# UCSB-NLP-Chang/Diffusion-SpaceTime-Attn

Hardware: AMD Instinct MI355X
Metric: images/sec at 512x512, 50 PLMS steps, 2 objects (higher is better)
Workload: dtype fp16; 1 GPU; SD-v1-4 UNet+VAE (synthetic weights), 512x512, 50 PLMS steps (51 CFG UNet calls), 2 objects, fixed blend weights (BASELINE configs[1]); global_batch=64, parallelism=prompt-parallel dp1, hipgraph=True, linear_weights=fp16, trunk_layout=NHWC, weight_broadcast_bytes=0

## Files before the change

diffusion-spacetime-attn_amd/csrc/sta_rowgemm.hip:

```cpp

#include <hip/hip_runtime.h>
#include <stdint.h>
#include "sta_xattn.h"
#include "sta_internal.h"
#include "sta_xattn_dev.h"
#include "sta_wring_dev.h"
#include "sta_xattn_proj3.h"

namespace {

constexpr int RG_C = 320;
constexpr int RG_NKS = RG_C / 32;
constexpr int RG_NRT = RG_C / 16;
constexpr int RG_NCH = RG_NRT / 2;
constexpr int RG_NW = 8;
constexpr int RG_CHUNK_FR = 2 * RG_NKS;
using RgRing = WRing<RG_NW, RG_CHUNK_FR>;
constexpr int RG_SLOT = RgRing::SLOT;
constexpr int RG_TAB = 3 * RG_C * 2;
constexpr int RG_LDS = 2 * RG_SLOT + RG_TAB;

__host__ __device__ constexpr int sfrag_channel(int f, int g, int j) {
  return f < 8 ? f * 40 + (j < 4 ? 4 * g + j : 16 + 4 * g + (j - 4)) : (4 * (f - 8) + g) * 40 + 32 + j;
}
// ... 98 lines not shown
    const T* xr = (const T*)p.x + row * RG_C + 8 * g;
    V8 xv[RG_NCH];
#pragma unroll
    for (int v = 0; v < RG_NCH; ++v) xv[v] = *(const V8*)(xr + 32 * v);
    float sum = 0.f;
#pragma unroll
    for (int v = 0; v < RG_NCH; ++v) {
      const V8 bs = *(const V8*)(tab + 32 * v + 8 * g);
      V8 o;
#pragma unroll
      for (int e = 0; e < 8; ++e) {
        const float t = acc[2 * v + (e >> 2)][e & 3] + (float)bs[e] + (float)xv[v][e];
        o[e] = (T)t;
        const float r = (float)o[e];
        acc[2 * v + (e >> 2)][e & 3] = r;
        sum += r;
      }
      *(V8*)((T*)p.s + row * RG_C + 32 * v + 8 * g) = o;
      __builtin_amdgcn_sched_barrier(0);
    }
    const float mean = bfly_sum(sum) * (1.0f / RG_C);
    float q = 0.f;
#pragma unroll
    for (int u = 0; u < RG_NRT; ++u)
#pragma unroll
      for (int r = 0; r < 4; ++r) {
        const float d = acc[u][r] - mean;
        q += d * d;
      }
    const float rstd = rsqrtf(bfly_sum(q) * (1.0f / RG_C) + p.eps);
#pragma unroll
    for (int v = 0; v < RG_NCH; ++v) {
      const V8 gm = *(const V8*)(tab + RG_C + 32 * v + 8 * g), bt = *(const V8*)(tab + 2 * RG_C + 32 * v + 8 * g);
      V8 o;
#pragma unroll
      for (int e = 0; e < 8; ++e) o[e] = (T)((acc[2 * v + (e >> 2)][e & 3] - mean) * rstd * (float)gm[e] + (float)bt[e]);
      if (p.y_qfrag) *(V8*)((char*)p.y + (size_t)row0 * RG_C * sizeof(T) + v * FRAG + lane * 16) = o;
      else *(V8*)((T*)p.y + row * RG_C + 32 * v + 8 * g) = o;
      __builtin_amdgcn_sched_barrier(0);
    }
    }
  }
  asm volatile("s_waitcnt vmcnt(0)" ::: "memory");
}

}

extern "C" {

size_t sta_to_out_ln_packed_wo_bytes(int C, int heads) {
  return (C == RG_C && heads == 8) ? (size_t)RG_NRT * RG_NKS * FRAG : 0;
}

int sta_to_out_ln_pack_wo(const void* wo, void* packed, int C, int heads, int kind, int dtype, void* stream) {
  g_sta_err[0] = 0;
  if (!wo || !packed) return sta_fail(STA_E_ARG, "null pointer");
  if (sta_to_out_ln_packed_wo_bytes(C, heads) == 0) return sta_fail(STA_E_UNSUP, "to_out + LayerNorm in out-fragment order: C = 320 with 8 heads only (C=%d heads=%d)", C, heads);
  if (dtype != STA_BF16 && dtype != STA_F16) return sta_fail(STA_E_UNSUP, "dtype %d", dtype);
  if (kind != 0 && kind != 1) return sta_fail(STA_E_ARG, "fragment kind %d (0: cross-attention out fragments, 1: self-attention out fragments)", kind);
  hipStream_t st = (hipStream_t)stream;
  return sta_by_dtype(dtype, [&](auto tag) {
    using T = decltype(tag);
    return sta_launch<pack_wo_ofrag_kernel<T>>("pack_wo_ofrag launch", dim3(RG_NRT * RG_NKS), dim3(64), 0, st, (const T*)wo, (T*)packed, kind);
  });
}

int sta_to_out_ln_ofrag(const void* blended_ofrag, const void* packed_wo, const void* bias, const void* x, const void* gamma,
                        const void* beta, void* s, void* y, long R, int C, int heads, float eps, int y_qfrag, int dtype, void* stream) {
  g_sta_err[0] = 0;
  if (!blended_ofrag || !packed_wo || !x || !gamma || !beta || !s || !y) return sta_fail(STA_E_ARG, "null pointer");
  if (sta_to_out_ln_packed_wo_bytes(C, heads) == 0) return sta_fail(STA_E_UNSUP, "to_out + LayerNorm in out-fragment order: C = 320 with 8 heads only (C=%d heads=%d)", C, heads);
  if (R <= 0 || R % 16) return sta_fail(STA_E_ARG, "to_out_ln_ofrag: R=%ld (need a positive multiple of 16 rows)", R);
  if ((size_t)R * C * 2 >= 0xfffffff0ull) return sta_fail(STA_E_UNSUP, "activations must stay below 4 GiB (R=%ld)", R);
  RG p{(const char*)blended_ofrag, (const char*)packed_wo, bias, gamma, beta, x, s, y, R, eps, y_qfrag ? 1 : 0};
  const long nblk = (R + 16 * RG_NW - 1) / (16 * RG_NW);
  const unsigned grid = (unsigned)(nblk < 256 ? nblk : 256);
  hipStream_t st = (hipStream_t)stream;
  return sta_by_dtype(dtype, [&](auto tag) {
    return sta_launch_lds<to_out_ln_ofrag_kernel<decltype(tag)>>("to_out_ln_ofrag launch", RG_LDS, dim3(grid), dim3(64 * RG_NW), RG_LDS, st, p);
  });
}

}
```

diffusion-spacetime-attn_amd/sta/fused.py:

```python

import torch

from . import lib

_DT = {torch.bfloat16: lib.STA_BF16, torch.float16: lib.STA_F16}
ENABLED = True
_hold = 0
TRACKED = False


class held:

    def __enter__(self):
        global _hold
        _hold += 1

    def __exit__(self, *exc):
        global _hold
        _hold -= 1


class tracked:

    def __init__(self, on=True):
# ... 427 lines not shown
    nb = max(1, min(B, CONV_MAX_BYTES // per_in))
    L = lib.load()
    slots = L.sta_conv3x3_s2_stats_slots(H, W) if stats else 0
    part = torch.empty((B + 1, slots, Cout, 2), dtype=torch.float32, device=x.device) if slots else None
    for b0 in range(0, B, nb):
        n = min(nb, B - b0)
        lib.check(L.sta_conv3x3_s2_nhwc(x.data_ptr() + b0 * per_in, w_packed.data_ptr(), z.data_ptr(), _ptr(bias), out.data_ptr() + b0 * per_out,
                                        0 if part is None else part.data_ptr() + b0 * slots * Cout * 8, n, H, W, Cin, Cout, _DT[x.dtype],
                                        _stream()), "sta_conv3x3_s2_nhwc")
    if part is not None and _version(out) is not None:
        out._sta_stats = (out._version, _finalize_stats(part, B, slots, Cout))
    return out


def vae_encode_step(h, quant_weight, quant_bias, n_post, n_enc, scale_factor, sqrt_a, sqrt_1ma, want_z0=False, want_xin=True):
    B, C, Hh, Ww = h.shape
    if C != 8 or not h.is_cuda or h.dtype not in _DT:
        raise ValueError("vae_encode_step: 16-bit CUDA h [B, 8, h, w], got %s %s" % (tuple(h.shape), h.dtype))
    h = h.contiguous(memory_format=torch.channels_last)
    qw = quant_weight.detach().reshape(8, 8).float().contiguous()
    qb = quant_bias.detach().float().contiguous()
    f = lambda t: t.detach().to(device=h.device, dtype=torch.float32).contiguous()
    n_post, n_enc = f(n_post), f(n_enc)
    if n_post.shape != (B, 4, Hh, Ww) or n_enc.shape != (B, 4, Hh, Ww):
        raise ValueError("vae_encode_step: noises must be [B, 4, h, w] = %s" % ((B, 4, Hh, Ww),))
    x = torch.empty((B, 4, Hh, Ww), dtype=torch.float32, device=h.device)
    z0 = torch.empty_like(x) if want_z0 else None
    xin = torch.empty((2 * B, 4, Hh, Ww), dtype=h.dtype, device=h.device) if want_xin else None
    lib.check(lib.load().sta_vae_encode_step(h.data_ptr(), qw.data_ptr(), qb.data_ptr(), n_post.data_ptr(), n_enc.data_ptr(), x.data_ptr(),
                                             _ptr(z0), _ptr(xin), B, Hh * Ww, float(scale_factor), float(sqrt_a), float(sqrt_1ma), _DT[h.dtype],
                                             _stream()), "sta_vae_encode_step")
    return x, z0, xin


CAT_IN_PLACE = True


def groupnorm_silu_cat(xa, xb, weight, bias, groups, eps, silu=True):
    B, Ca = xa.shape[0], xa.shape[1]
    C = Ca + xb.shape[1]
    HW = xa.numel() // (B * Ca)
    L = lib.load()
    y = torch.empty((B, C) + tuple(xa.shape[2:]), dtype=xa.dtype, device=xa.device, memory_format=torch.channels_last)
    sa, sb = (_producer_stats(xa), _producer_stats(xb)) if GN_STATS_FROM_PRODUCER else (None, None)
    if sa is not None and sb is not None:
        lib.check(L.sta_groupnorm_silu_nhwc_cstats(xa.data_ptr(), xb.data_ptr(), Ca, sa.data_ptr(), sb.data_ptr(), None, weight.data_ptr(),
                                                   bias.data_ptr(), y.data_ptr(), B, C, HW, groups, float(eps), int(bool(silu)), _DT[xa.dtype],
                                                   _stream()), "sta_groupnorm_silu_nhwc_cstats")
        return y
    ws = torch.empty(L.sta_groupnorm_nhwc_workspace_bytes(B, HW, groups) // 4, dtype=torch.float32, device=xa.device)
    lib.check(L.sta_groupnorm_silu_nhwc_cat(xa.data_ptr(), xb.data_ptr(), Ca, None, weight.data_ptr(), bias.data_ptr(), y.data_ptr(),
                                            ws.data_ptr(), B, C, HW, groups, float(eps), int(bool(silu)), _DT[xa.dtype], _stream()),
              "sta_groupnorm_silu_nhwc_cat")
    return y


def cat_supported(xa, xb, groups, skip_weight):
    if not (CAT_IN_PLACE and usable(xa) and is_nhwc(xa) and is_nhwc(xb) and xa.dtype == xb.dtype and xa.shape[0] == xb.shape[0]
            and xa.shape[2:] == xb.shape[2:]):
        return False
    Ca, C = xa.shape[1], xa.shape[1] + xb.shape[1]
    if Ca % 64 or C % 8 or C % groups or (C // groups < 8 and C // groups != 4) or C > 4096 or groups > 64:
        return False
    rows = xa.numel() // Ca
    return (LINEAR_ROWS and rows >= LINEAR_MIN_ROWS and skip_weight.dtype == xa.dtype
            and bool(lib.load().sta_linear_rows_supported(rows, C, skip_weight.shape[0])))


def linear_rows_cat(xa, xb, w_packed, N, bias=None, res=None):
    Ka, Kb = xa.shape[-1], xb.shape[-1]
    R = xa.numel() // Ka
    assert xa.is_contiguous() and xb.is_contiguous() and xb.numel() // Kb == R and Ka % 64 == 0
    out = torch.empty(xa.shape[:-1] + (N,), dtype=xa.dtype, device=xa.device)
    if bias is not None:
        bias = bias.to(xa.dtype).contiguous()
    z = _zeros_page(xa.device, 2 * (Ka + Kb))
    lib.check(lib.load().sta_linear_rows_cat(xa.data_ptr(), xb.data_ptr(), Ka, w_packed.data_ptr(), z.data_ptr(), _ptr(bias), _ptr(res),
                                             out.data_ptr(), R, Ka + Kb, N, _DT[xa.dtype], _stream()), "sta_linear_rows_cat")
    return out


LINEAR_ROWS = True
LINEAR_MIN_ROWS = 4096


_retired_pages = []


def _zeros_page(device, nbytes):
    z = _conv_zeros.get(device)
    if z is None or z.numel() < nbytes:
        if z is not None:
            _retired_pages.append(z)
        z = _conv_zeros[device] = torch.zeros(max(nbytes, 16384), dtype=torch.uint8, device=device)
    return z


def linear_rows_supported(x, weight):
    if not (LINEAR_ROWS and x.is_cuda and x.dtype in _DT and not torch.is_grad_enabled() and ENABLED and not _hold and weight.dtype == x.dtype):
        return False
    K = x.shape[-1]
    R = x.numel() // K
    return R >= LINEAR_MIN_ROWS and x.is_contiguous() and bool(lib.load().sta_linear_rows_supported(R, K, weight.shape[0]))


def pack_linear_weight(weight):
    N, K = weight.shape[0], weight.shape[1]
    L = lib.load()
    n = L.sta_linear_rows_packed_w_bytes(K, N)
    if n == 0 or not weight.is_cuda:
        raise ValueError("linear_rows: a CUDA weight [N %% 160 == 0 or N %% 128 == 0, K %% 64 == 0]; got %s" % (tuple(weight.shape),))
    w = weight.detach()
    buf = torch.empty(n, dtype=torch.uint8, device=w.device)
    lib.check(L.sta_linear_rows_pack_w(w.data_ptr(), w.stride(0), w.stride(1), buf.data_ptr(), K, N, _DT[w.dtype], _stream()), "sta_linear_rows_pack_w")
    return buf


def linear_rows(x, w_packed, N, bias=None, res=None, stats_rows=None):
    K = x.shape[-1]
    R = x.numel() // K
    out = torch.empty(x.shape[:-1] + (N,), dtype=x.dtype, device=x.device)
    if res is not None:
        assert res.numel() == out.numel() and res.dtype == x.dtype and res.is_contiguous()
    if bias is not None:
        bias = bias.to(x.dtype).contiguous()
    z = _zeros_page(x.device, 2 * K)
    if stats_rows and stats_rows % 256 == 0 and R % stats_rows == 0:
        n_img, slots = R // stats_rows, stats_rows // 64
        part = torch.empty((n_img + 1, slots, N, 2), dtype=torch.float32, device=x.device)
        lib.check(lib.load().sta_linear_rows_stats(x.data_ptr(), w_packed.data_ptr(), z.data_ptr(), _ptr(bias), _ptr(res), out.data_ptr(),
                                                   part.data_ptr(), stats_rows, R, K, N, _DT[x.dtype], _stream()), "sta_linear_rows_stats")
        if _version(out) is not None:
            out._sta_stats = (out._version, _finalize_stats(part, n_img, slots, N))
        return out
    lib.check(lib.load().sta_linear_rows(x.data_ptr(), w_packed.data_ptr(), z.data_ptr(), _ptr(bias), _ptr(res), out.data_ptr(), R, K, N,
                                         _DT[x.dtype], _stream()), "sta_linear_rows")
    return out


def packed_linear_weight(owner, key_obj, weight):
    return cached_image(owner, ("linear", id(key_obj)), (weight,), lambda: pack_linear_weight(weight))


def linear_module(lin, x, res=None):
    if linear_rows_supported(x, lin.weight) and (res is None or res.is_contiguous()):
        return linear_rows(x, packed_linear_weight(lin, lin, lin.weight), lin.weight.shape[0], bias=lin.bias, res=res)
    y = torch.nn.functional.linear(x, lin.weight, lin.bias)
    return y if res is None else y + res


def add_bias_nchw(a, b=None, bias=None):
    B, C = a.shape[0], a.shape[1]
    HW = a.numel() // (B * C)
    if (C % 8 if is_nhwc(a) else HW % 8):
        t = a if b is None else a + b
        return t if bias is None else t + bias[None, :, None, None]
    y = torch.empty_like(a)
    if is_nhwc(a):
        if b is not None and not is_nhwc(b):
            b = b.contiguous(memory_format=torch.channels_last)
        lib.check(lib.load().sta_add_bias_rows(a.data_ptr(), _ptr(b), _ptr(bias), y.data_ptr(), B * HW, C, _DT[a.dtype], _stream()),
                  "sta_add_bias_rows")
        return y
    if b is not None and not b.is_contiguous():
        b = b.contiguous()
    lib.check(lib.load().sta_add_bias_nchw(a.data_ptr(), _ptr(b), _ptr(bias), y.data_ptr(), B, C, HW, _DT[a.dtype], _stream()),
              "sta_add_bias_nchw")
    return y


def tracked_usable(x):
    return (TRACKED and ENABLED and x.is_cuda and x.dtype in _DT and torch.is_grad_enabled()
            and (is_nhwc(x) if x.dim() == 4 else x.is_contiguous()))


class GroupNormSiLUFn(torch.autograd.Function):

    @staticmethod
    def forward(ctx, x, add, weight, bias, groups, eps, silu):
        B, C = x.shape[0], x.shape[1]
        HW = x.numel() // (B * C)
        L = lib.load()
        add = None if add is None else add.float().contiguous()
        y = torch.empty_like(x)
        ws = torch.empty(L.sta_groupnorm_nhwc_workspace_bytes(B, HW, groups) // 4, dtype=torch.float32, device=x.device)
        lib.check(L.sta_groupnorm_silu_nhwc(x.data_ptr(), _ptr(add), weight.data_ptr(), bias.data_ptr(), y.data_ptr(), ws.data_ptr(),
                                            B, C, HW, groups, float(eps), int(bool(silu)), _DT[x.dtype], _stream()), "sta_groupnorm_silu_nhwc")
        ctx.save_for_backward(x, add, weight, bias, ws)
        ctx.cfg = (B, C, HW, groups, float(eps), int(bool(silu)))
        return y

    @staticmethod
    def backward(ctx, dy):
        x, add, weight, bias, ws = ctx.saved_tensors
        B, C, HW, groups, eps, silu = ctx.cfg
        if not is_nhwc(dy):
            dy = dy.contiguous(memory_format=torch.channels_last)
        dx = torch.empty_like(x)
        wsb = torch.empty_like(ws)
        lib.check(lib.load().sta_groupnorm_silu_nhwc_bwd(x.data_ptr(), _ptr(add), weight.data_ptr(), bias.data_ptr(), dy.data_ptr(),
                                                         dx.data_ptr(), ws.data_ptr(), wsb.data_ptr(), B, C, HW, groups, eps, silu,
                                                         _DT[x.dtype], _stream()), "sta_groupnorm_silu_nhwc_bwd")
        return dx, None, None, None, None, None, None


def groupnorm_silu_tracked(x, weight, bias, groups, eps, add=None, silu=True):
    C = x.shape[1]
    if add is not None and add.requires_grad:
        raise RuntimeError("the pre-add of the fused GroupNorm carries no gradient (timestep embedding)")
    if not is_nhwc(x) or C % 8 or (C // groups < 8 and C // groups != 4) or C > 4096 or groups > 64:
        h = x if add is None else x + add.to(x.dtype)[:, :, None, None]
        h = torch.nn.functional.group_norm(h, groups, weight, bias, eps)
        return torch.nn.functional.silu(h) if silu else h
    return GroupNormSiLUFn.apply(x, add, weight, bias, groups, eps, silu)


class GegluFn(torch.autograd.Function):
    @staticmethod
    def forward(ctx, h):
        ctx.save_for_backward(h)
        return geglu(h)

    @staticmethod
    def backward(ctx, dy):
# ... 98 lines not shown
```

diffusion-spacetime-attn_amd/sta/lib.py:

```python
import ctypes
import glob
import os
import shutil
import subprocess

_HERE = os.path.dirname(os.path.abspath(__file__))
PKG_ROOT = os.path.dirname(_HERE)
REPO_ROOT = os.path.dirname(PKG_ROOT)
CSRC = os.path.join(PKG_ROOT, "csrc")
INCLUDE = os.path.join(REPO_ROOT, "include")
LIB_PATH = os.path.join(CSRC, "libsta_xattn.so")
SOURCES = [os.path.join(CSRC, n) for n in ("sta_xattn.hip", "sta_xattn_bwd.hip", "sta_xattn_proj.hip", "sta_xattn_proj3.hip", "sta_rowgemm.hip", "sta_ffgemm.hip", "sta_lnqkv.hip", "sta_conv.hip", "sta_gemm.hip", "sta_selfattn.hip", "sta_selfattn_bwd.hip", "sta_unet.hip", "sta_unet_bwd.hip", "sta_fp8.hip", "sta_mxfp8.hip", "sta_sampler.hip", "sta_encode.hip", "sta_clip.hip", "sta_inpaint.hip")]
INCLUDED_SOURCES = {"sta_xattn_maps_bwd.hip": "sta_xattn_bwd.hip", "sta_guide.hip": "sta_sampler.hip", "sta_window.hip": "sta_sampler.hip"}

PER_SOURCE_FLAGS = {"sta_selfattn.hip": ["-mllvm", "-amdgpu-mfma-vgpr-form", "-ffinite-math-only"],
                    "sta_selfattn_bwd.hip": ["-mllvm", "-amdgpu-mfma-vgpr-form", "-ffinite-math-only"],
                    "sta_xattn.hip": ["-ffinite-math-only"], "sta_xattn_bwd.hip": ["-ffinite-math-only"], "sta_xattn_proj.hip": ["-ffinite-math-only"],
                    "sta_xattn_proj3.hip": ["-ffinite-math-only"], "sta_rowgemm.hip": ["-ffinite-math-only"], "sta_ffgemm.hip": ["-ffinite-math-only"], "sta_conv.hip": ["-ffinite-math-only"], "sta_gemm.hip": ["-ffinite-math-only"]}

NO_SPILL_KERNELS = {"sta_ffgemm.hip": ("ff_geglu_qfrag_kernel",), "sta_conv.hip": ("ELb1EEEvNS_2CVE",),
                    "sta_sampler.hip": ("window_split_kernel", "window_fuse_kernel", "sampler_step_windows_kernel",
                                        "sampler_step_windows_masked_kernel", "window_blend_kernel")}

STA_BF16, STA_F16 = 0, 1
STA_MX8_GEGLU, STA_MX8_MX_OUT = 1, 2
OPT_FWD_KERNEL, OPT_STAGED_TILES, OPT_STAGED_WAVES, OPT_STAGED_QT, OPT_HEAD_MAJOR, OPT_SPLIT_QT, OPT_SELFATTN_32, OPT_PROJ_PAIR, OPT_SELFATTN_WAVES, OPT_SELFATTN_PIPE, OPT_PROJ_LL2, OPT_BWD_KERNEL, OPT_BWD_SLOTS, OPT_BWD_WAVES = range(14)
FWD_STAGED, FWD_SPLIT = 1, 2
MAX_KEYS, MAX_HEAD_DIM, MAX_OBJECTS = 80, 160, 8
P3_STATS_WORDS = 8
MAX_READOUTS = 16
MAX_WINDOW_OFFSETS, STA_SRC_F32 = 16, 2

_vp, _i, _f, _sz, _l = ctypes.c_void_p, ctypes.c_int, ctypes.c_float, ctypes.c_size_t, ctypes.c_long
SYMBOLS = {
    "sta_version": (_i, []),
    "sta_last_error": (ctypes.c_char_p, []),
    "sta_built_with": (ctypes.c_char_p, []),
    "sta_set_option": (_i, [_i, _i]),
    "sta_xattn_packed_kv_bytes": (_sz, [_i, _i, _i]),
    "sta_xattn_pack_kv": (_i, [_vp, _vp, _vp, _i, _i, _i, _i, _i, _vp]),
    "sta_xattn_fwd": (_i, [_vp, _vp, _vp, _vp, _vp, _vp, _i, _i, _i, _i, _i, _i, _f, _i, _vp]),
    "sta_xattn_token_maps": (_i, [_vp, _vp, _vp, _vp, _vp, _i, _i, _i, _i, _i, _i, _i, _f, _i, _i, _vp]),
    "sta_xattn_token_maps_bwd": (_i, [_vp, _vp, _vp, _vp, _vp, _vp, _i, _i, _i, _i, _i, _i, _i, _f, _i, _vp]),
    "sta_xattn_fwd_proj_supported": (_i, [_i, _i, _i, _i]),
    "sta_xattn_fwd_proj_locals_from_l2": (_i, [_i, _i, _i, _i]),
    "sta_xattn_packed_wq_bytes": (_sz, [_i, _i]),
    "sta_xattn_pack_wq": (_i, [_vp, _vp, _i, _i, _i, _vp]),
    "sta_xattn_packed_kv_proj_bytes": (_sz, [_i, _i, _i]),
    "sta_xattn_pack_kv_proj": (_i, [_vp, _vp, _vp, _i, _i, _i, _i, _i, _vp]),
    "sta_xattn_fwd_proj": (_i, [_vp, _vp, _vp, _vp, _vp, _vp, _i, _i, _i, _i, _i, _i, _f, _i, _vp]),
    "sta_xattn_fwd_proj_qfrag_supported": (_i, [_i, _i, _i, _i, _i, _i]),
    "sta_xattn_fwd_proj_ex": (_i, [_vp, _vp, _vp, _vp, _vp, _vp, _i, _i, _i, _i, _i, _i, _f, _i, _i, _vp, _vp]),
    "sta_xattn_fwd_proj_qfrag": (_i, [_vp, _vp, _vp, _vp, _vp, _vp, _i, _i, _i, _i, _i, _i, _f, _i, _vp]),
    "sta_xattn_fwd_proj_qfrag_ofrag": (_i, [_vp, _vp, _vp, _vp, _vp, _vp, _i, _i, _i, _i, _i, _i, _f, _i, _vp]),
    "sta_to_out_ln_packed_wo_bytes": (_sz, [_i, _i]),
    "sta_to_out_ln_pack_wo": (_i, [_vp, _vp, _i, _i, _i, _i, _vp]),
    "sta_to_out_ln_ofrag": (_i, [_vp, _vp, _vp, _vp, _vp, _vp, _vp, _vp, _l, _i, _i, _f, _i, _i, _vp]),
    "sta_selfattn_fwd_sfrag": (_i, [_vp, _vp, _vp, _vp, _i, _i, _i, _i, _i, _i, _l, _l, _f, _i, _vp]),
    "sta_xattn_bwd_workspace_bytes": (_sz, [_i, _i, _i, _i]),
    "sta_xattn_bwd": (_i, [_vp, _vp, _vp, _vp, _vp, _vp, _vp, _vp, _i, _i, _i, _i, _i, _i, _f, _i, _vp]),
    "sta_selfattn_fwd": (_i, [_vp, _vp, _vp, _vp, _i, _i, _i, _i, _i, _i, _l, _l, _f, _i, _vp]),
    "sta_selfattn_fwd_optimistic": (_i, [_vp, _vp, _vp, _vp, _vp, _i, _i, _i, _i, _i, _i, _l, _l, _f, _i, _i, _vp]),
    "sta_selfattn_optimistic_supported": (_i, [_i, _i, _i, _f, _i]),
    "sta_selfattn_optimistic_flags_bytes": (ctypes.c_size_t, [_i, _i, _i]),
    "sta_selfattn_fwd_lse": (_i, [_vp, _vp, _vp, _vp, _vp, _i, _i, _i, _i, _i, _i, _l, _l, _f, _i, _vp]),
    "sta_selfattn_bwd": (_i, [_vp] * 13 + [_i, _i, _i, _i, _i, _i, _f, _i, _vp]),
    "sta_groupnorm_silu": (_i, [_vp, _vp, _vp, _vp, _vp, _i, _i, _i, _i, _f, _i, _i, _vp]),
    "sta_geglu": (_i, [_vp, _vp, _l, _i, _i, _vp]),
    "sta_add_layernorm": (_i, [_vp, _vp, _vp, _vp, _vp, _vp, _vp, _l, _i, _f, _i, _vp]),
    "sta_add_layernorm_qfrag": (_i, [_vp, _vp, _vp, _vp, _vp, _vp, _vp, _l, _i, _f, _i, _vp]),
    "sta_ff_geglu_packed_w_bytes": (_sz, [_i, _i]),
    "sta_ff_geglu_pack_w": (_i, [_vp, _vp, _i, _i, _i, _vp]),
    "sta_ff_geglu_qfrag": (_i, [_vp, _vp, _vp, _vp, _l, _i, _i, _i, _i, _vp]),
    "sta_ff_geglu_c640_packed_w_bytes": (_sz, [_i, _i]),
    "sta_ff_geglu_c640_pack_w": (_i, [_vp, _vp, _i, _i, _i, _vp]),
    "sta_ff_geglu_c640_qfrag": (_i, [_vp, _vp, _vp, _vp, _l, _i, _i, _i, _i, _vp]),
    "sta_ff_out_packed_w_bytes": (_sz, [_i, _i]),
    "sta_ff_out_pack_w": (_i, [_vp, _vp, _i, _i, _i, _vp]),
    "sta_ff_out_res_hfrag": (_i, [_vp, _vp, _vp, _vp, _vp, _l, _i, _i, _i, _vp]),
    "sta_ln_qkv_packed_w_bytes": (_sz, [_i]),
    "sta_ln_qkv_pack_w": (_i, [_vp, _vp, _vp, _i, _i, _vp]),
    "sta_ln_qkv": (_i, [_vp] * 9 + [_l, _i, _f, _i, _vp]),
    "sta_conv3x3_nhwc_supported": (_i, [_i, _i, _i, _i, _i]),
    "sta_conv3x3_packed_w_bytes": (_sz, [_i, _i]),
    "sta_conv3x3_pack_w": (_i, [_vp, _l, _l, _l, _l, _vp, _i, _i, _i, _vp]),
    "sta_conv3x3_nhwc": (_i, [_vp, _vp, _vp, _vp, _vp, _vp, _vp, _i, _i, _i, _i, _i, _i, _i, _vp]),
    "sta_conv3x3_up2_nhwc_supported": (_i, [_i, _i, _i, _i, _i]),
    "sta_conv3x3_up2_stats_slots": (_i, [_i, _i]),
    "sta_conv3x3_up2_packed_w_bytes": (_sz, [_i, _i]),
    "sta_conv3x3_up2_pack_w": (_i, [_vp, _l, _l, _l, _l, _vp, _i, _i, _i, _vp]),
    "sta_conv3x3_up2_nhwc": (_i, [_vp, _vp, _vp, _vp, _vp, _vp, _vp, _i, _i, _i, _i, _i, _i, _vp]),
    "sta_linear_rows_supported": (_i, [_l, _i, _i]),
    "sta_linear_rows_packed_w_bytes": (_sz, [_i, _i]),
    "sta_linear_rows_pack_w": (_i, [_vp, _l, _l, _vp, _i, _i, _i, _vp]),
    "sta_linear_rows": (_i, [_vp, _vp, _vp, _vp, _vp, _vp, _l, _i, _i, _i, _vp]),
    "sta_conv3x3_stats_slots": (_i, [_i, _i]),
    "sta_stats_finalize": (_i, [_vp, _vp, _i, _i, _i, _vp]),
    "sta_linear_rows_stats": (_i, [_vp, _vp, _vp, _vp, _vp, _vp, _vp, _l, _l, _i, _i, _i, _vp]),
    "sta_groupnorm_silu_nhwc_cstats": (_i, [_vp, _vp, _i, _vp, _vp, _vp, _vp, _vp, _vp, _i, _i, _i, _i, _f, _i, _i, _vp]),
    "sta_linear_rows_cat": (_i, [_vp, _vp, _i, _vp, _vp, _vp, _vp, _vp, _l, _i, _i, _i, _vp]),
    "sta_groupnorm_silu_nhwc_cat": (_i, [_vp, _vp, _i, _vp, _vp, _vp, _vp, _vp, _i, _i, _i, _i, _f, _i, _i, _vp]),
    "sta_add_bias_nchw": (_i, [_vp, _vp, _vp, _vp, _i, _i, _i, _i, _vp]),
    "sta_groupnorm_nhwc_workspace_bytes": (_sz, [_i, _i, _i]),
    "sta_groupnorm_silu_nhwc": (_i, [_vp, _vp, _vp, _vp, _vp, _vp, _i, _i, _i, _i, _f, _i, _i, _vp]),
    "sta_add_bias_rows": (_i, [_vp, _vp, _vp, _vp, _l, _i, _i, _vp]),
    "sta_quant_rows_fp8": (_i, [_vp, _vp, _vp, _l, _i, _i, _vp]),
    "sta_mx8_quant_rows": (_i, [_vp, _vp, _vp, _l, _i, _i, _vp]),
    "sta_mx8_gemm": (_i, [_vp, _vp, _vp, _vp, _vp, _vp, _vp, _vp, _l, _i, _i, _l, _i, _i, _vp]),
    "sta_groupnorm_silu_nhwc_bwd": (_i, [_vp, _vp, _vp, _vp, _vp, _vp, _vp, _vp, _i, _i, _i, _i, _f, _i, _i, _vp]),
    "sta_geglu_bwd": (_i, [_vp, _vp, _vp, _l, _i, _i, _vp]),
    "sta_layernorm_bwd": (_i, [_vp, _vp, _vp, _vp, _vp, _l, _i, _f, _i, _vp]),
    "sta_sampler_step": (_i, [_vp] * 7 + [_l, _l] + [_f] * 8 + [_i, _vp]),
    "sta_sampler_step_bwd": (_i, [_vp] * 5 + [_l, _l] + [_f] * 7 + [_i, _vp]),
    "sta_conv3x3_s2_nhwc_supported": (_i, [_i, _i, _i, _i, _i]),
    "sta_conv3x3_s2_stats_slots": (_i, [_i, _i]),
    "sta_conv3x3_s2_nhwc": (_i, [_vp] * 6 + [_i] * 6 + [_vp]),
    "sta_vae_encode_step": (_i, [_vp] * 8 + [_l, _l, _f, _f, _f, _i, _vp]),
    "sta_clip_views": (_i, [_vp] * 4 + [_i] * 5 + [_vp]),
    "sta_clip_views_bwd": (_i, [_vp] * 4 + [_i] * 5 + [_vp]),
    "sta_sampler_step_masked": (_i, [_vp] * 10 + [_l, _l, _l] + [_f] * 10 + [_i, _vp]),
    "sta_sampler_step_masked_bwd": (_i, [_vp] * 6 + [_l, _l, _l] + [_f] * 7 + [_i, _vp]),
    "sta_latent_blend": (_i, [_vp] * 6 + [_l, _l, _l, _f, _f, _i, _vp]),
    "sta_image_composite": (_i, [_vp] * 4 + [_l, _l, _i, _vp]),
    "sta_image_composite_bwd": (_i, [_vp] * 4 + [_l, _l, _i, _vp]),
    "sta_latent_guide": (_i, [_vp] * 7 + [_l, _l, _l, _i, _f, _i, _vp]),
    "sta_window_split": (_i, [_vp, _vp, _l] + [_i] * 6 + [_vp, _vp] + [_i] * 3 + [_vp]),
    "sta_window_fuse": (_i, [_vp, _vp, _l] + [_i] * 5 + [_vp, _vp, _i, _i, _vp]),
    "sta_sampler_step_windows": (_i, [_vp] * 7 + [_l] + [_i] * 5 + [_vp, _vp, _i] + [_f] * 8 + [_i, _vp]),
    "sta_sampler_step_windows_masked": (_i, [_vp] * 10 + [_l] + [_i] * 5 + [_vp, _vp, _i] + [_f] * 10 + [_i, _vp]),
    "sta_window_blend": (_i, [_vp] * 6 + [_l] + [_i] * 5 + [_vp, _vp, _i, _f, _f, _i, _vp]),
}


class StaLibraryError(RuntimeError):
    pass


def _stale():
    if not os.path.exists(LIB_PATH):
        return True
    t = os.path.getmtime(LIB_PATH)
    deps = SOURCES + [os.path.join(CSRC, n) for n in INCLUDED_SOURCES] + [os.path.join(_HERE, "isa_lint.py")] + glob.glob(os.path.join(INCLUDE, "*.h")) + glob.glob(os.path.join(CSRC, "*.h"))
    return any(os.path.exists(d) and os.path.getmtime(d) > t for d in deps)


LINT_LOG = os.path.join(CSRC, ".isa_lint.log")


def _llvm_bin(hipcc):
    for root in (os.environ.get("ROCM_PATH"), os.path.dirname(os.path.dirname(os.path.realpath(hipcc))), "/opt/rocm"):
        if root and os.path.exists(os.path.join(root, "lib", "llvm", "bin", "clang")):
            return os.path.join(root, "lib", "llvm", "bin")
    raise StaLibraryError("no lib/llvm/bin/clang beside %s (set ROCM_PATH)" % hipcc)


def _hipcc_headline(hipcc):
    ver = subprocess.run([hipcc, "--version"], capture_output=True, text=True).stdout.strip().splitlines()
    return ver[0] if ver else "hipcc ?"


def _run(cmd):
    r = subprocess.run(cmd, capture_output=True, text=True)
    if r.returncode != 0:
        raise StaLibraryError("build step failed: %s\n%s" % (" ".join(cmd), r.stdout + r.stderr))


_META_KEYS = ("vgpr_count", "vgpr_spill_count", "sgpr_spill_count", "private_segment_fixed_size", "group_segment_fixed_size")


def kernel_metadata(text):
    out, cur, inside = {}, None, False
    for line in text.splitlines():
        if line.startswith("amdhsa.kernels:"):
            inside = True
        elif inside and line[:1] not in (" ", ""):
            inside = False
        if not inside:
            continue
# ... 148 lines not shown
```

include/sta_unet.h:

```cpp
#ifndef STA_UNET_H
#define STA_UNET_H

#include <stddef.h>
#include <stdint.h>

#ifdef __cplusplus
extern "C" {
#endif

int sta_groupnorm_silu(const void* x, const float* add, const void* gamma, const void* beta, void* y,
                       int B, int C, int HW, int G, float eps, int silu, int dtype, void* stream);

int sta_geglu(const void* x, void* y, long R, int D, int dtype, void* stream);

int sta_add_layernorm(const void* x, const void* f, const void* bias, const void* gamma, const void* beta,
                      void* s, void* y, long R, int C, float eps, int dtype, void* stream);

int sta_add_layernorm_qfrag(const void* x, const void* f, const void* bias, const void* gamma, const void* beta,
                            void* s, void* y, long R, int C, float eps, int dtype, void* stream);

size_t sta_ff_geglu_packed_w_bytes(int C, int inner);
int sta_ff_geglu_pack_w(const void* w, void* packed, int C, int inner, int dtype, void* stream);
int sta_ff_geglu_qfrag(const void* y_qfrag, const void* packed_w, const void* bias, void* h, long R, int C, int inner,
                       int h_frag, int dtype, void* stream);
size_t sta_ff_out_packed_w_bytes(int C, int inner);
int sta_ff_out_pack_w(const void* w, void* packed, int C, int inner, int dtype, void* stream);
int sta_ff_out_res_hfrag(const void* h_frag, const void* packed_w, const void* bias, const void* x, void* out, long R, int C,
                         int inner, int dtype, void* stream);

size_t sta_ff_geglu_c640_packed_w_bytes(int C, int inner);
int sta_ff_geglu_c640_pack_w(const void* w, void* packed, int C, int inner, int dtype, void* stream);
int sta_ff_geglu_c640_qfrag(const void* y_qfrag, const void* packed_w, const void* bias, void* h, long R, int C, int inner,
                            int max_workgroups, int dtype, void* stream);

size_t sta_ln_qkv_packed_w_bytes(int C);
int sta_ln_qkv_pack_w(const void* wqk, const void* wv, void* packed, int C, int dtype, void* stream);
int sta_ln_qkv(const void* x, const void* bias, const void* gamma, const void* beta, const void* packed_w, void* s, void* y_dbg,
               void* qk, void* vt, long R, int C, float eps, int dtype, void* stream);

int sta_conv3x3_nhwc_supported(int B, int H, int W, int Cin, int Cout);
int sta_conv3x3_stats_slots(int H, int W);
int sta_stats_finalize(const float* partial, float* stats, int B, int slots, int C, void* stream);
size_t sta_conv3x3_packed_w_bytes(int Cin, int Cout);
int sta_conv3x3_pack_w(const void* w, long so, long si, long sy, long sx, void* packed, int Cin, int Cout, int dtype, void* stream);
int sta_conv3x3_nhwc(const void* x, const void* packed_w, const void* zeros, const void* bias, const void* res, void* out, float* stats, int B,
                     int H, int W, int Cin, int Cout, int up2, int dtype, void* stream);

int sta_conv3x3_up2_nhwc_supported(int B, int H, int W, int Cin, int Cout);
int sta_conv3x3_up2_stats_slots(int H, int W);
size_t sta_conv3x3_up2_packed_w_bytes(int Cin, int Cout);
int sta_conv3x3_up2_pack_w(const void* w, long so, long si, long sy, long sx, void* packed, int Cin, int Cout, int dtype, void* stream);
int sta_conv3x3_up2_nhwc(const void* x, const void* packed_w, const void* zeros, const void* bias, const void* res, void* out, float* stats, int B,
                         int H, int W, int Cin, int Cout, int dtype, void* stream);

int sta_linear_rows_supported(long R, int K, int N);
size_t sta_linear_rows_packed_w_bytes(int K, int N);
int sta_linear_rows_pack_w(const void* w, long sn, long sk, void* packed, int K, int N, int dtype, void* stream);
int sta_linear_rows(const void* x, const void* packed_w, const void* zeros, const void* bias, const void* res, void* out, long R, int K,
                    int N, int dtype, void* stream);
int sta_linear_rows_stats(const void* x, const void* packed_w, const void* zeros, const void* bias, const void* res, void* out, float* stats,
                          long rows_per_image, long R, int K, int N, int dtype, void* stream);
int sta_linear_rows_cat(const void* xa, const void* xb, int Ka, const void* packed_w, const void* zeros, const void* bias, const void* res,
                        void* out, long R, int K, int N, int dtype, void* stream);

int sta_add_bias_nchw(const void* a, const void* b, const void* bias, void* y, int B, int C, int HW,
                      int dtype, void* stream);

size_t sta_groupnorm_nhwc_workspace_bytes(int B, int HW, int G);
int sta_groupnorm_silu_nhwc(const void* x, const float* add, const void* gamma, const void* beta, void* y,
                            void* workspace, int B, int C, int HW, int G, float eps, int silu, int dtype, void* stream);
int sta_groupnorm_silu_nhwc_cat(const void* xa, const void* xb, int Ca, const float* add, const void* gamma, const void* beta, void* y,
                                void* workspace, int B, int C, int HW, int G, float eps, int silu, int dtype, void* stream);
int sta_groupnorm_silu_nhwc_cstats(const void* xa, const void* xb, int Ca, const float* stats_a, const float* stats_b, const float* add,
                                   const void* gamma, const void* beta, void* y, int B, int C, int HW, int G, float eps, int silu, int dtype,
                                   void* stream);

int sta_add_bias_rows(const void* a, const void* b, const void* bias, void* y, long rows, int C, int dtype, void* stream);

int sta_quant_rows_fp8(const void* x, void* xq, float* scale, long rows, int C, int dtype, void* stream);

enum { STA_MX8_GEGLU = 1, STA_MX8_MX_OUT = 2 };
int sta_mx8_quant_rows(const void* x, void* xq, void* xs, long rows, int K, int dtype, void* stream);
int sta_mx8_gemm(const void* p, const void* ps, const void* q, const void* qs, void* out, void* out_scale, const void* bias,
                 const float* col_scale, long M, int N, int K, long ldo, int flags, int dtype, void* stream);

int sta_groupnorm_silu_nhwc_bwd(const void* x, const float* add, const void* gamma, const void* beta, const void* dy, void* dx,
                                const void* fwd_workspace, void* bwd_workspace, int B, int C, int HW, int G, float eps, int silu,
                                int dtype, void* stream);
int sta_conv3x3_s2_nhwc_supported(int B, int H, int W, int Cin, int Cout);
int sta_conv3x3_s2_stats_slots(int H, int W);
int sta_conv3x3_s2_nhwc(const void* x, const void* packed_w, const void* zeros, const void* bias, void* out, float* stats, int B, int H, int W,
                        int Cin, int Cout, int dtype, void* stream);

int sta_vae_encode_step(const void* h, const float* quant_w, const float* quant_b, const float* n_post, const float* n_enc, float* x, float* z0,
                        void* xin, long B, long hw, float scale_factor, float sqrt_a, float sqrt_1ma, int dtype, void* stream);

int sta_geglu_bwd(const void* x, const void* dy, void* dx, long R, int D, int dtype, void* stream);
int sta_layernorm_bwd(const void* s, const void* gamma, const void* dy, const void* dres, void* ds, long R, int C, float eps,
                      int dtype, void* stream);

int sta_sampler_step(const void* eps, const float* x, const float* m_prev, const float* noise, float* x_next, float* m, void* xin,
                     long b, long n, float scale, float sigma_t, float alpha_t, float c_x, float c_m, float c_p, float c_e, float c_n,
                     int dtype, void* stream);
int sta_sampler_step_bwd(const float* g_xn, const float* g_m, float* g_x, void* g_eps, float* g_mprev, long b, long n, float scale,
                         float sigma_t, float alpha_t, float c_x, float c_m, float c_p, float c_e, int dtype, void* stream);

int sta_sampler_step_masked(const void* eps, const float* x, const float* m_prev, const float* noise, const float* x0, const float* keep,
                            const float* qnoise, float* x_next, float* m, void* xin, long b, long n, long hw, float scale, float sigma_t,
                            float alpha_t, float c_x, float c_m, float c_p, float c_e, float c_n, float q_a, float q_b, int dtype,
                            void* stream);
int sta_sampler_step_masked_bwd(const float* g_xn, const float* g_m, const float* keep, float* g_x, void* g_eps, float* g_mprev, long b,
                                long n, long hw, float scale, float sigma_t, float alpha_t, float c_x, float c_m, float c_p, float c_e,
                                int dtype, void* stream);
int sta_latent_blend(const float* x, const float* x0, const float* keep, const float* noise, float* x_out, void* xin, long b, long n, long hw,
                     float q_a, float q_b, int dtype, void* stream);
int sta_image_composite(const void* dec, const float* orig, const float* keep_px, void* out, long b, long hw, int dtype, void* stream);
int sta_image_composite_bwd(const void* g, const void* dec, const float* keep_px, void* g_dec, long b, long hw, int dtype, void* stream);

int sta_latent_guide(const void* g, const float* x, const float* keep, const float* step, float* x_out, void* xin, float* stats, long b, long n,
                     long hw, int normalize, float inv_scale, int dtype, void* stream);

#define STA_MAX_WINDOW_OFFSETS 16
#define STA_SRC_F32 2
int sta_window_split(const void* src, void* xin, long P, int rows, int C, int Hc, int Wc, int ny, int nx, const int* oy, const int* ox, int s,
                     int src_dtype, int dtype, void* stream);
int sta_window_fuse(const void* eps, void* out, long P, int C, int Hc, int Wc, int ny, int nx, const int* oy, const int* ox, int s, int dtype,
                    void* stream);
int sta_sampler_step_windows(const void* eps, const float* x, const float* m_prev, const float* noise, float* x_next, float* m, void* xin, long P,
                             int C, int Hc, int Wc, int ny, int nx, const int* oy, const int* ox, int s, float scale, float sigma_t,
                             float alpha_t, float c_x, float c_m, float c_p, float c_e, float c_n, int dtype, void* stream);
int sta_sampler_step_windows_masked(const void* eps, const float* x, const float* m_prev, const float* noise, const float* x0,
                                    const float* keep, const float* qnoise, float* x_next, float* m, void* xin, long P, int C, int Hc, int Wc,
                                    int ny, int nx, const int* oy, const int* ox, int s, float scale, float sigma_t, float alpha_t, float c_x,
                                    float c_m, float c_p, float c_e, float c_n, float q_a, float q_b, int dtype, void* stream);
int sta_window_blend(const float* x, const float* x0, const float* keep, const float* noise, float* x_out, void* xin, long P, int C, int Hc,
                     int Wc, int ny, int nx, const int* oy, const int* ox, int s, float q_a, float q_b, int dtype, void* stream);

int sta_clip_views(const float* img, const int* boxes, const int* boxes_host, void* out, int B, int H, int W, int n_views, int out_dtype,
                   void* stream);
int sta_clip_views_bwd(const void* dout, const int* boxes, const int* boxes_host, float* dimg, int B, int H, int W, int n_views, int dtype,
                       void* stream);

#ifdef __cplusplus
}
#endif
#endif
// ... 1 lines not shown
```

Measured before the change: 10.04 images/s.

## Add specialized 320x320 row GEMM kernel with LDS-resident weight halves

Adds a dedicated kernel for 320-in/320-out row linears (proj_in/proj_out at the top UNet level). Each block keeps one half of the packed weight resident in LDS for its whole lifetime and walks contiguous tile ranges per wave, double-buffering activation loads and fusing bias, residual add and per-image GroupNorm partial statistics. The Python linear path sends eligible 320x320 calls to it instead of the generic linear_rows kernel. The aim is to cut repeated weight staging and improve reuse on the largest-resolution linears, at the cost of an extra packed weight copy and a different stats slot layout.

```diff
diff --git a/diffusion-spacetime-attn_amd/csrc/sta_rowgemm.hip b/diffusion-spacetime-attn_amd/csrc/sta_rowgemm.hip
--- a/diffusion-spacetime-attn_amd/csrc/sta_rowgemm.hip
+++ b/diffusion-spacetime-attn_amd/csrc/sta_rowgemm.hip
@@ -204,3 +204,5 @@
 }
 
 }
+
+#include "sta_rows320.hip"
diff --git a/diffusion-spacetime-attn_amd/csrc/sta_rows320.hip b/diffusion-spacetime-attn_amd/csrc/sta_rows320.hip
--- /dev/null
+++ b/diffusion-spacetime-attn_amd/csrc/sta_rows320.hip
@@ -0,0 +1,243 @@
+
+
+#include <hip/hip_runtime.h>
+#include <stdint.h>
+#include "sta_xattn.h"
+#include "sta_unet.h"
+#include "sta_internal.h"
+#include "sta_xattn_dev.h"
+#include "sta_wring_dev.h"
+
+namespace {
+
+constexpr int R3_C = 320;
+constexpr int R3_NKS = R3_C / 32;
+constexpr int R3_HALF = R3_C / 2;
+constexpr int R3_NRT = R3_HALF / 16;
+constexpr int R3_NPAIR = R3_NRT / 2;
+constexpr int R3_WFR = R3_NRT * R3_NKS;
+constexpr int R3_NW = 8;
+constexpr int R3_LDS = R3_WFR * FRAG + R3_HALF * 2;
+constexpr int R3_ROW = R3_C * 2;
+constexpr int R3_MAX_PAIRS = 128;
+
+template <typename T>
+__global__ __launch_bounds__(64) void pack_rows320_w_kernel(const T* __restrict__ w, long sn, long sk, T* __restrict__ packed) {
+  const int fr = blockIdx.x;
+  const int f = fr % R3_NKS, t = (fr / R3_NKS) % R3_NRT, half = fr / R3_WFR;
+  const int lane = threadIdx.x, g = lane >> 4, c = lane & 15;
+  const T* src = w + (size_t)(R3_HALF * half + frag_sigma(t, c)) * sn + (size_t)(32 * f + 8 * g) * sk;
+  typename Tr<T>::V8 x;
+#pragma unroll
+  for (int j = 0; j < 8; ++j) x[j] = src[j * sk];
+  *(typename Tr<T>::V8*)(packed + (size_t)fr * (FRAG / 2) + lane * 8) = x;
+}
+
+struct R3 {
+  const void* x;
+  const char* w;
+  const void* bias;
+  const void* res;
+  void* out;
+  float* stats;
+  long tiles;
+  int ch;
+  int slots;
+  int npairs;
+};
+
+struct R3Cut {
+  int ch, slots, npairs;
+};
+R3Cut r3_cut(long tiles, long tiles_img) {
+  long npairs = (tiles + R3_NW - 1) / R3_NW;
+  if (npairs > R3_MAX_PAIRS) npairs = R3_MAX_PAIRS;
+  long ch = (tiles + npairs * R3_NW - 1) / (npairs * R3_NW);
+  int slots = 0;
+  if (tiles_img) {
+    const long least = tiles_img < 4 ? tiles_img : 4;
+    if (ch < least) ch = least;
+    while (ch < tiles_img && tiles_img % ch) ++ch;
+    if (ch > tiles_img) ch = tiles_img;
+    slots = (int)(tiles_img / ch);
+  }
+  const long nranges = (tiles + ch - 1) / ch;
+  npairs = (nranges + R3_NW - 1) / R3_NW;
+  return R3Cut{(int)ch, slots, (int)(npairs < R3_MAX_PAIRS ? npairs : R3_MAX_PAIRS)};
+}
+
+template <typename T, bool RES, bool ST>
+__global__ __launch_bounds__(64 * R3_NW, 2) void rows320_kernel(const R3 p) {
+  using V8 = typename Tr<T>::V8;
+  const int lane = threadIdx.x & 63;
+  const int wv = __builtin_amdgcn_readfirstlane(threadIdx.x >> 6);
+  const int g = lane >> 4, c16 = lane & 15;
+  const int half = (blockIdx.x >> 3) & 1, pair = (int)(blockIdx.x >> 4) * 8 + (blockIdx.x & 7);
+  if (pair >= p.npairs) return;
+  {
+    const __amdgpu_buffer_rsrc_t w_srd = make_srd(p.w + (size_t)half * R3_WFR * FRAG, (unsigned)(R3_WFR * FRAG));
+    for (int f = wv; f < R3_WFR; f += R3_NW)
+      __builtin_amdgcn_raw_ptr_buffer_load_lds(w_srd, (__attribute__((address_space(3))) void*)(smem + f * FRAG), 16, (unsigned)lane * 16u,
+                                               (unsigned)(f * FRAG), 0, 0);
+    T* tab = (T*)(smem + R3_WFR * FRAG);
+    for (int i = threadIdx.x; i < R3_HALF; i += 64 * R3_NW) tab[i] = p.bias ? ((const T*)p.bias)[R3_HALF * half + i] : (T)0.0f;
+    asm volatile("s_waitcnt vmcnt(0)" ::: "memory");
+    __syncthreads();
+  }
+  const V8* wf = (const V8*)(smem + lane * 16);
+  const T* tab = (const T*)(smem + R3_WFR * FRAG) + 8 * g;
+  const unsigned bytes = (unsigned)(p.tiles * 16 * R3_ROW);
+  const __amdgpu_buffer_rsrc_t x_srd = make_srd(p.x, bytes), r_srd = make_srd(RES ? p.res : p.x, bytes), o_srd = make_srd(p.out, bytes);
+  const unsigned voff = (unsigned)(c16 * R3_ROW + g * 16);
+  float ssum[ST ? R3_NPAIR : 1][8], ssq[ST ? R3_NPAIR : 1][8];
+  long t1 = 0;
+
+  constexpr bool PF = !ST;
+  auto load_b = [&](V8 (&b)[R3_NKS], const unsigned vo) __attribute__((always_inline)) {
+#pragma unroll
+    for (int f = 0; f < R3_NKS; ++f) b[f] = srd_load16<V8>(x_srd, vo, 64u * f);
+  };
+  auto tile = [&](const long t, V8 (&b)[R3_NKS], V8 (&bn)[R3_NKS]) __attribute__((always_inline)) {
+    const unsigned base = (unsigned)(t * (16 * R3_ROW));
+    const unsigned eo = base + voff + (unsigned)(half * R3_HALF * 2);
+    if constexpr (!PF) load_b(b, base + voff);
+    V8 rv[RES ? R3_NPAIR : 1];
+    if constexpr (RES) {
+#pragma unroll
+      for (int v = 0; v < R3_NPAIR; ++v) rv[v] = srd_load16<V8>(r_srd, eo, 64u * v);
+    }
+    if constexpr (PF) load_b(bn, t + 1 < t1 ? base + (unsigned)(16 * R3_ROW) + voff : SRD_DROP);
+    V8 wa[2][R3_NKS / 2];
+    auto fetch = [&](int h, V8 (&a)[R3_NKS / 2]) __attribute__((always_inline)) {
+#pragma unroll
+      for (int i = 0; i < R3_NKS / 2; ++i) a[i] = wf[(h * (R3_NKS / 2) + i) * 64];
+    };
+    fetch(0, wa[0]);
+    f32x4 acc[2];
+    sta_static_for<2 * R3_NRT>([&](auto h_tag) __attribute__((always_inline)) {
+      constexpr int H = decltype(h_tag)::value;
+      constexpr int U = H >> 1, K0 = (H & 1) * (R3_NKS / 2);
+      if constexpr (H + 1 < 2 * R3_NRT) fetch(H + 1, wa[(H + 1) & 1]);
+      __builtin_amdgcn_sched_barrier(0);
+      f32x4 a = {0.f, 0.f, 0.f, 0.f};
+      if constexpr (K0 != 0) a = acc[U & 1];
+#pragma unroll
+      for (int i = 0; i < R3_NKS / 2; ++i) a = Tr<T>::mfma(wa[H & 1][i], b[K0 + i], a);
+      acc[U & 1] = a;
+      __builtin_amdgcn_sched_barrier(0);
+      if constexpr ((H & 3) == 3) {
+        constexpr int V = H >> 2;
+        const V8 bs = *(const V8*)(tab + 32 * V);
+        V8 o;
+#pragma unroll
+        for (int e = 0; e < 8; ++e) {
+          float r32 = acc[e >> 2][e & 3] + (float)bs[e];
+          if constexpr (RES) r32 += (float)rv[V][e];
+          o[e] = (T)r32;
+          if constexpr (ST) {
+            const float r = (float)o[e];
+            ssum[V][e] += r;
+            ssq[V][e] += r * r;
+          }
+        }
+        __builtin_amdgcn_raw_buffer_store_b128(__builtin_bit_cast(u32x4, o), o_srd, eo + 64u * V, 0, 0);
+      }
+    });
+  };
+
+  const long nranges = (p.tiles + p.ch - 1) / p.ch;
+  for (long range = (long)pair * R3_NW + wv; range < nranges; range += (long)p.npairs * R3_NW) {
+  const long t0 = range * p.ch;
+  t1 = t0 + p.ch < p.tiles ? t0 + p.ch : p.tiles;
+  if constexpr (ST) {
+#pragma unroll
+    for (int v = 0; v < R3_NPAIR; ++v)
+#pragma unroll
+      for (int e = 0; e < 8; ++e) { ssum[v][e] = 0.f; ssq[v][e] = 0.f; }
+  }
+  if constexpr (PF) {
+    V8 b0[R3_NKS], b1[R3_NKS];
+    load_b(b0, (unsigned)(t0 * (16 * R3_ROW)) + voff);
+    for (long t = t0; t < t1; t += 2) {
+      tile(t, b0, b1);
+      if (t + 1 < t1) tile(t + 1, b1, b0);
+    }
+  } else {
+    V8 b[R3_NKS];
+    for (long t = t0; t < t1; ++t) tile(t, b, b);
+  }
+
+  if constexpr (ST) {
+    float* dst = p.stats + ((size_t)range * R3_C + R3_HALF * half + 8 * g) * 2;
+#pragma unroll
+    for (int v = 0; v < R3_NPAIR; ++v) {
+      float s[8], q[8];
+#pragma unroll
+      for (int e = 0; e < 8; ++e) {
+        s[e] = ssum[v][e];
+        q[e] = ssq[v][e];
+#pragma unroll
+        for (int o = 8; o > 0; o >>= 1) {
+          s[e] += __shfl_xor(s[e], o);
+          q[e] += __shfl_xor(q[e], o);
+        }
+      }
+      if (c16 == 0) {
+#pragma unroll
+        for (int e = 0; e < 8; e += 2) *(f32x4*)(dst + 64 * v + 2 * e) = f32x4{s[e], q[e], s[e + 1], q[e + 1]};
+      }
+    }
+  }
+  }
+}
+
+}
+
+extern "C" {
+
+int sta_rows320_supported(long R, int K, int N) {
+  return K == R3_C && N == R3_C && R > 0 && R % 16 == 0 && (size_t)R * R3_ROW < 0xfffffff0ull;
+}
+
+size_t sta_rows320_packed_w_bytes(int K, int N) { return (K == R3_C && N == R3_C) ? (size_t)2 * R3_WFR * FRAG : 0; }
+
+int sta_rows320_pack_w(const void* w, long sn, long sk, void* packed, int K, int N, int dtype, void* stream) {
+  g_sta_err[0] = 0;
+  if (!w || !packed) return sta_fail(STA_E_ARG, "null pointer");
+  if (sta_rows320_packed_w_bytes(K, N) == 0) return sta_fail(STA_E_UNSUP, "rows320: K = N = 320 only (K=%d N=%d)", K, N);
+  hipStream_t st = (hipStream_t)stream;
+  return sta_by_dtype(dtype, [&](auto tag) {
+    using T = decltype(tag);
+    return sta_launch<pack_rows320_w_kernel<T>>("pack_rows320_w launch", dim3(2 * R3_WFR), dim3(64), 0, st, (const T*)w, sn, sk, (T*)packed);
+  });
+}
+
+int sta_rows320_stats_slots(long R, long rows_per_image) {
+  if (!sta_rows320_supported(R, R3_C, R3_C) || rows_per_image <= 0 || rows_per_image % 16 || R % rows_per_image) return 0;
+  return r3_cut(R / 16, rows_per_image / 16).slots;
+}
+
+int sta_rows320(const void* x, const void* packed_w, const void* bias, const void* res, void* out, float* stats, long rows_per_image, long R,
+                int dtype, void* stream) {
+  g_sta_err[0] = 0;
+  if (!x || !packed_w || !out) return sta_fail(STA_E_ARG, "null pointer");
+  if (!sta_rows320_supported(R, R3_C, R3_C)) return sta_fail(STA_E_UNSUP, "rows320: R=%ld (need a positive multiple of 16 rows below 4 GiB)", R);
+  if (dtype != STA_BF16 && dtype != STA_F16) return sta_fail(STA_E_UNSUP, "dtype %d", dtype);
+  if (stats && sta_rows320_stats_slots(R, rows_per_image) == 0)
+    return sta_fail(STA_E_ARG, "rows320: rows_per_image=%ld (need a multiple of 16 dividing R=%ld)", rows_per_image, R);
+  const R3Cut cut = r3_cut(R / 16, stats ? rows_per_image / 16 : 0);
+  R3 p{x, (const char*)packed_w, bias, res, out, stats, R / 16, cut.ch, cut.slots, cut.npairs};
+  const dim3 grid(16 * ((cut.npairs + 7) / 8));
+  hipStream_t st = (hipStream_t)stream;
+  return sta_by_dtype(dtype, [&](auto tag) {
+    using T = decltype(tag);
+    const char* const what = "rows320 launch";
+    auto launch = [&](auto res_tag, auto st_tag) {
+      return sta_launch_lds<rows320_kernel<T, decltype(res_tag)::value, decltype(st_tag)::value>>(what, R3_LDS, grid, dim3(64 * R3_NW), R3_LDS, st, p);
+    };
+    if (res) return stats ? launch(std::true_type{}, std::true_type{}) : launch(std::true_type{}, std::false_type{});
+    return stats ? launch(std::false_type{}, std::true_type{}) : launch(std::false_type{}, std::false_type{});
+  });
+}
+
+}
diff --git a/diffusion-spacetime-attn_amd/sta/fused.py b/diffusion-spacetime-attn_amd/sta/fused.py
--- a/diffusion-spacetime-attn_amd/sta/fused.py
+++ b/diffusion-spacetime-attn_amd/sta/fused.py
@@ -533,6 +533,7 @@
 
 LINEAR_ROWS = True
 LINEAR_MIN_ROWS = 4096
+ROWS320 = True
 
 
 _retired_pages = []
@@ -555,7 +556,19 @@
     return R >= LINEAR_MIN_ROWS and x.is_contiguous() and bool(lib.load().sta_linear_rows_supported(R, K, weight.shape[0]))
 
 
-def pack_linear_weight(weight):
+def pack_rows320_weight(weight):
+    N, K = weight.shape[0], weight.shape[1]
+    L = lib.load()
+    n = L.sta_rows320_packed_w_bytes(K, N)
+    if n == 0 or not weight.is_cuda:
+        return None
+    w = weight.detach()
+    buf = torch.empty(n, dtype=torch.uint8, device=w.device)
+    lib.check(L.sta_rows320_pack_w(w.data_ptr(), w.stride(0), w.stride(1), buf.data_ptr(), K, N, _DT[w.dtype], _stream()), "sta_rows320_pack_w")
+    return buf
+
+
+def pack_linear_weight(weight, rows320=True):
     N, K = weight.shape[0], weight.shape[1]
     L = lib.load()
     n = L.sta_linear_rows_packed_w_bytes(K, N)
@@ -564,6 +577,9 @@
     w = weight.detach()
     buf = torch.empty(n, dtype=torch.uint8, device=w.device)
     lib.check(L.sta_linear_rows_pack_w(w.data_ptr(), w.stride(0), w.stride(1), buf.data_ptr(), K, N, _DT[w.dtype], _stream()), "sta_linear_rows_pack_w")
+    w320 = pack_rows320_weight(weight) if rows320 and ROWS320 else None
+    if w320 is not None:
+        buf._sta_rows320 = w320
     return buf
 
 
@@ -575,8 +591,20 @@
         assert res.numel() == out.numel() and res.dtype == x.dtype and res.is_contiguous()
     if bias is not None:
         bias = bias.to(x.dtype).contiguous()
+    want_stats = bool(stats_rows and stats_rows % 256 == 0 and R % stats_rows == 0)
+    w320 = getattr(w_packed, "_sta_rows320", None) if ROWS320 else None
+    if w320 is not None and lib.load().sta_rows320_supported(R, K, N):
+        L = lib.load()
+        n_img = R // stats_rows if want_stats else 0
+        slots = L.sta_rows320_stats_slots(R, stats_rows) if want_stats else 0
+        part = torch.empty((n_img + 1, slots, N, 2), dtype=torch.float32, device=x.device) if want_stats else None
+        lib.check(L.sta_rows320(x.data_ptr(), w320.data_ptr(), _ptr(bias), _ptr(res), out.data_ptr(), _ptr(part), stats_rows if want_stats else 0,
+                                R, _DT[x.dtype], _stream()), "sta_rows320")
+        if want_stats and _version(out) is not None:
+            out._sta_stats = (out._version, _finalize_stats(part, n_img, slots, N))
+        return out
     z = _zeros_page(x.device, 2 * K)
-    if stats_rows and stats_rows % 256 == 0 and R % stats_rows == 0:
+    if want_stats:
         n_img, slots = R // stats_rows, stats_rows // 64
         part = torch.empty((n_img + 1, slots, N, 2), dtype=torch.float32, device=x.device)
         lib.check(lib.load().sta_linear_rows_stats(x.data_ptr(), w_packed.data_ptr(), z.data_ptr(), _ptr(bias), _ptr(res), out.data_ptr(),
@@ -590,7 +618,11 @@
 
 
 def packed_linear_weight(owner, key_obj, weight):
-    return cached_image(owner, ("linear", id(key_obj)), (weight,), lambda: pack_linear_weight(weight))
+    wp = cached_image(owner, ("linear", id(key_obj)), (weight,), lambda: pack_linear_weight(weight, rows320=False))
+    w320 = cached_image(owner, ("rows320", id(key_obj)), (weight,), lambda: pack_rows320_weight(weight)) if ROWS320 else None
+    if w320 is not None:
+        wp._sta_rows320 = w320
+    return wp
 
 
 def linear_module(lin, x, res=None):
diff --git a/diffusion-spacetime-attn_amd/sta/lib.py b/diffusion-spacetime-attn_amd/sta/lib.py
--- a/diffusion-spacetime-attn_amd/sta/lib.py
+++ b/diffusion-spacetime-attn_amd/sta/lib.py
@@ -11,7 +11,8 @@
 INCLUDE = os.path.join(REPO_ROOT, "include")
 LIB_PATH = os.path.join(CSRC, "libsta_xattn.so")
 SOURCES = [os.path.join(CSRC, n) for n in ("sta_xattn.hip", "sta_xattn_bwd.hip", "sta_xattn_proj.hip", "sta_xattn_proj3.hip", "sta_rowgemm.hip", "sta_ffgemm.hip", "sta_lnqkv.hip", "sta_conv.hip", "sta_gemm.hip", "sta_selfattn.hip", "sta_selfattn_bwd.hip", "sta_unet.hip", "sta_unet_bwd.hip", "sta_fp8.hip", "sta_mxfp8.hip", "sta_sampler.hip", "sta_encode.hip", "sta_clip.hip", "sta_inpaint.hip")]
-INCLUDED_SOURCES = {"sta_xattn_maps_bwd.hip": "sta_xattn_bwd.hip", "sta_guide.hip": "sta_sampler.hip", "sta_window.hip": "sta_sampler.hip"}
+INCLUDED_SOURCES = {"sta_xattn_maps_bwd.hip": "sta_xattn_bwd.hip", "sta_guide.hip": "sta_sampler.hip", "sta_window.hip": "sta_sampler.hip",
+                    "sta_rows320.hip": "sta_rowgemm.hip"}
 
 PER_SOURCE_FLAGS = {"sta_selfattn.hip": ["-mllvm", "-amdgpu-mfma-vgpr-form", "-ffinite-math-only"],
                     "sta_selfattn_bwd.hip": ["-mllvm", "-amdgpu-mfma-vgpr-form", "-ffinite-math-only"],
@@ -94,6 +95,11 @@
     "sta_linear_rows_packed_w_bytes": (_sz, [_i, _i]),
     "sta_linear_rows_pack_w": (_i, [_vp, _l, _l, _vp, _i, _i, _i, _vp]),
     "sta_linear_rows": (_i, [_vp, _vp, _vp, _vp, _vp, _vp, _l, _i, _i, _i, _vp]),
+    "sta_rows320_supported": (_i, [_l, _i, _i]),
+    "sta_rows320_packed_w_bytes": (_sz, [_i, _i]),
+    "sta_rows320_pack_w": (_i, [_vp, _l, _l, _vp, _i, _i, _i, _vp]),
+    "sta_rows320_stats_slots": (_i, [_l, _l]),
+    "sta_rows320": (_i, [_vp, _vp, _vp, _vp, _vp, _vp, _l, _l, _i, _vp]),
     "sta_conv3x3_stats_slots": (_i, [_i, _i]),
     "sta_stats_finalize": (_i, [_vp, _vp, _i, _i, _i, _vp]),
     "sta_linear_rows_stats": (_i, [_vp, _vp, _vp, _vp, _vp, _vp, _vp, _l, _l, _i, _i, _i, _vp]),
diff --git a/include/sta_unet.h b/include/sta_unet.h
--- a/include/sta_unet.h
+++ b/include/sta_unet.h
@@ -62,6 +62,13 @@
                           long rows_per_image, long R, int K, int N, int dtype, void* stream);
 int sta_linear_rows_cat(const void* xa, const void* xb, int Ka, const void* packed_w, const void* zeros, const void* bias, const void* res,
                         void* out, long R, int K, int N, int dtype, void* stream);
+
+int sta_rows320_supported(long R, int K, int N);
+size_t sta_rows320_packed_w_bytes(int K, int N);
+int sta_rows320_pack_w(const void* w, long sn, long sk, void* packed, int K, int N, int dtype, void* stream);
+int sta_rows320_stats_slots(long R, long rows_per_image);
+int sta_rows320(const void* x, const void* packed_w, const void* bias, const void* res, void* out, float* stats, long rows_per_image, long R,
+                int dtype, void* stream);
 
 int sta_add_bias_nchw(const void* a, const void* b, const void* bias, void* y, int B, int C, int HW,
                       int dtype, void* stream);
```

New measurement: 10.11 images/s (median of 6 runs). No clear change (+0.7%).
